# OpenPPL/ppl.llm.serving

Measured on AMD Instinct MI355X. Metric: decode tokens/sec, LLaMA-7B int8 (W8A16), max-running-batch 1024, higher is better.
Workload: dtype fp16 activations, int8 weights (W8A16), int8-g8 KV, fp32 accumulate

## Files before the change

include/pplhip.h:

```cpp
#ifndef PPLHIP_H_
#define PPLHIP_H_

#include <stdint.h>
#include <stddef.h>

#ifdef __cplusplus
extern "C" {
#endif

#define PPLHIP_API __attribute__((visibility("default")))

typedef enum pplhip_status {
    PPLHIP_SUCCESS = 0,
    PPLHIP_OTHER_ERROR = -1,
    PPLHIP_INVALID_VALUE = -2,
    PPLHIP_OUT_OF_MEMORY = -3,
    PPLHIP_DEVICE_RUNTIME_ERROR = -4,
    PPLHIP_DEVICE_MEMORY_ERROR = -5,
    PPLHIP_NOT_FOUND = -6,
    PPLHIP_UNSUPPORTED = -7
} pplhip_status;

typedef struct pplhip_model_desc {
    int32_t hidden_dim;
// ... 358 lines not shown


PPLHIP_API int pplhip_op_rmsnorm_form(int64_t rows, int32_t hidden, int32_t quant, int32_t wide_max_rows, char* buf, int32_t len);

PPLHIP_API int pplhip_op_rmsnorm_ex(void* stream, const void* x, const void* skip, const void* w, float eps, int64_t rows, int32_t hidden,
                                    const int64_t* gather_seq_starts, void* out, void* residual_out, void* q, float* sx, int32_t q_fp8,
                                    const float* slab_ws, int32_t slab_splits, const void* slab_scale, int64_t slab_M);

PPLHIP_API int pplhip_op_gather_last_rows(void* stream, const void* x, const int64_t* seq_starts, int64_t B, int32_t hidden, void* out);

PPLHIP_API int pplhip_op_rope_kv_write_ex(void* stream, void* qkv, const float* cos_sin, const pplhip_kv_view* kv, const int64_t* seq_starts,
                                          const int64_t* start_pos, const int64_t* cache_indices, int64_t max_pages, int64_t B, int64_t t0,
                                          int64_t T, int32_t num_heads, const float* slab_ws, int32_t slab_splits, const void* slab_scale,
                                          int64_t slab_M);

PPLHIP_API int pplhip_op_linear_defer(void* stream, const void* x, const void* w, const void* scale, int32_t wq_bit, int32_t group,
                                      int64_t M, int32_t N, int32_t K, void* y, int64_t ldy, void* ws, uint64_t ws_bytes, int32_t dry_run,
                                      int32_t* splits, const void** slab_scale, char* route, int32_t route_len);

PPLHIP_API int pplhip_op_attention(void* stream, const void* qkv, const pplhip_kv_view* kv,
                                   const int64_t* seq_starts, const int64_t* start_pos,
                                   const int64_t* cache_indices, int64_t max_pages, int64_t B, int64_t T,
                                   int64_t decoding_batches, int64_t max_seq_len, int64_t max_kv_len,
                                   int32_t num_heads, int32_t split_k, void* workspace, uint64_t workspace_bytes,
                                   void* out);

enum { PPLHIP_COMM_ALLREDUCE = 0, PPLHIP_COMM_ALLREDUCE_NORM = 1, PPLHIP_COMM_ALLGATHER = 2 };
typedef struct pplhip_comm_item {
    int32_t kind, channel;
    uint32_t epoch_advance;
// ... 28 lines not shown
```

ppl.llm.serving_amd/csrc/k_attn_decode.hip:

```cpp
#include <stdlib.h>
#include <hip/hip_ext.h>
#include "k_attn_decode_dev.h"

namespace pplhip {

template <int QBIT, int D>
__global__ void attn_decode_kernel(const uint16_t* __restrict__ qkv, KvAddr kv, const int64_t* __restrict__ seq_starts,
                                   const int64_t* __restrict__ start_pos, const int64_t* __restrict__ cache_indices,
                                   int64_t max_pages, int H, int Hkv, int split, float* __restrict__ workspace,
                                   uint16_t* __restrict__ out) {
    extern __shared__ __attribute__((aligned(16))) float smem[];
    attn_decode_body<QBIT, D>(qkv, kv, seq_starts, start_pos, cache_indices, max_pages, H, Hkv, split, workspace, out, (int)blockIdx.x,
                              (int64_t)blockIdx.y, (int)blockIdx.z, (int)(blockDim.x >> 6), smem);
}

template <int D>
__global__ void attn_decode_reduce_kernel(const float* __restrict__ workspace, int split, uint16_t* __restrict__ out) {
    const int64_t bh = blockIdx.x;
    const float* ws = workspace + bh * (int64_t)split * (D + 2);
    for (int d = threadIdx.x; d < D; d += blockDim.x) {
        const LseRow r = lse_merge(ws, split, D + 2, D, d);
        out[bh * D + d] = f2h(r.o / r.l);
    }
}

hipError_t launch_attn_reduce(hipStream_t s, const float* ws, int nsplit, int64_t n_row_heads, int D, uint16_t* out) {
    if (D != 128 && D != 64 && D != 32) return hipErrorInvalidValue;
    dispatch_int<128, 64, 32>(D, [&](auto DD) {
        hipLaunchKernelGGL((attn_decode_reduce_kernel<DD>), dim3((unsigned)n_row_heads), dim3(DD < 64 ? 64 : DD), 0, s, ws, nsplit, out);
    });
    return hipGetLastError();
}

size_t attn_decode_workspace_bytes(int64_t nb, int H, int D, int split) {
    return split > 1 ? (size_t)nb * H * split * (D + 2) * sizeof(float) : 0;
}

template <int QBIT, int D>
static hipError_t launch_decode_t(hipStream_t s, const uint16_t* qkv, const KvAddr& kv, const int64_t* seq_starts,
                                  const int64_t* start_pos, const int64_t* cache_indices, int64_t max_pages, int64_t nb,
                                  int H, int Hkv, int split, int threads, float* workspace, uint16_t* out, hipEvent_t t0,
                                  hipEvent_t t1) {
    const int nw = threads / 64;
    const size_t lds = (size_t)nw * (D + 2) * sizeof(float);
    if (t0 && t1)
        hipExtLaunchKernelGGL((attn_decode_kernel<QBIT, D>), dim3(H, (unsigned)nb, split), dim3(threads), lds, s, t0, t1, 0, qkv, kv,
                              seq_starts, start_pos, cache_indices, max_pages, H, Hkv, split, workspace, out);
    else
        hipLaunchKernelGGL((attn_decode_kernel<QBIT, D>), dim3(H, (unsigned)nb, split), dim3(threads), lds, s, qkv, kv,
                           seq_starts, start_pos, cache_indices, max_pages, H, Hkv, split, workspace, out);
    const hipError_t e = hipGetLastError();
    if (e != hipSuccess || split == 1) return e;
    return launch_attn_reduce(s, workspace, split, nb * H, D, out);
}

hipError_t launch_attn_decode(hipStream_t s, const uint16_t* qkv, const KvAddr& kv, int kv_fmt,
                              const int64_t* seq_starts, const int64_t* start_pos, const int64_t* cache_indices,
                              int64_t max_pages, int64_t nb, int H, int Hkv, int D, int64_t max_kv_len, int split,
                              int threads, float* workspace, uint16_t* out, hipEvent_t t0, hipEvent_t t1) {
    if (nb == 0) return hipSuccess;
    static const int forced_tpb = tune_int("PPLHIP_ATTN_TPB", 0);
    if (forced_tpb) threads = forced_tpb;
    if (threads < 64 || threads > 64 * DEC_MAX_WAVES || threads % 64) return hipErrorInvalidValue;
    if (threads < D) threads = D;
    if (split < 1) split = 1;
    static const bool no_gqa = tune_set("PPLHIP_ATTN_NOGQA");
    if (attn_decode_gqa_supported(kv_fmt, H, Hkv, D) && !no_gqa) {
        hipError_t e = launch_attn_decode_gqa(s, qkv, kv, kv_fmt, seq_starts, start_pos, cache_indices, max_pages, nb, H,
                                              Hkv, D, split, workspace, out, t0, t1);
        if (e != hipSuccess || split == 1) return e;
        return launch_attn_reduce(s, workspace, split, nb * H, D, out);
    }
    if ((kv_fmt != KV_FP16 && kv_fmt != KV_I8G8 && kv_fmt != KV_FP8 && kv_fmt != KV_I4G32) || (D != 128 && D != 64 && D != 32)) return hipErrorInvalidValue;
    hipError_t e = hipSuccess;
    dispatch_int<KV_I8G8, KV_FP16, KV_FP8, KV_I4G32>(kv_fmt, [&](auto QB) {
        dispatch_int<128, 64, 32>(D, [&](auto DD) {
            e = launch_decode_t<QB, DD>(s, qkv, kv, seq_starts, start_pos, cache_indices, max_pages, nb, H, Hkv, split, threads, workspace,
                                        out, t0, t1);
        });
    });
    return e;
}

}
```

ppl.llm.serving_amd/csrc/k_attn_decode_dev.h:

```cpp
#pragma once
#include "k_attn_dev.h"

namespace pplhip {

constexpr int DEC_UNROLL = 4;
constexpr int DEC_MAX_WAVES = 8;

template <int QBIT, int D>
__device__ __forceinline__ void attn_decode_body(const uint16_t* __restrict__ qkv, const KvAddr& kv, const int64_t* __restrict__ seq_starts,
                                                 const int64_t* __restrict__ start_pos, const int64_t* __restrict__ cache_indices,
                                                 int64_t max_pages, int H, int Hkv, int split, float* __restrict__ workspace,
                                                 uint16_t* __restrict__ out, int hq, int64_t b, int sp, int nw, float* smem) {
    using C = AttnCfg<QBIT, D>;
    constexpr int CH = C::CH, LPT = C::LPT, TPW = C::TPW;

    const int hk = hq / (H / Hkv);
    const int lane = threadIdx.x & 63;
    const int wave = threadIdx.x >> 6;
    const int g = lane / LPT;
    const int c = lane - g * LPT;
    const int ch0 = c * CH;

    const int64_t kv_len = start_pos[b] + 1;
    const int64_t per = (kv_len + split - 1) / split;
    const int64_t tbeg = sp * per;
    const int64_t tend = (tbeg + per < kv_len) ? tbeg + per : kv_len;

    const uint16_t* qrow = qkv + seq_starts[b] * (int64_t)(H + 2 * Hkv) * D + (int64_t)hq * D + ch0;
    float q[CH];
    if constexpr (CH == 32) {
#pragma unroll
        for (int i = 0; i < 4; ++i) unpack8(*reinterpret_cast<const uint4*>(qrow + 8 * i), q + 8 * i);
    } else if constexpr (CH == 16) {
        unpack8(*reinterpret_cast<const uint4*>(qrow), q);
        unpack8(*reinterpret_cast<const uint4*>(qrow + 8), q + 8);
    } else {
        unpack8(*reinterpret_cast<const uint4*>(qrow), q);
    }
    float qsum[C::NG > 0 ? C::NG : 1];
    if constexpr (QBIT == 8) {
#pragma unroll
        for (int gi = 0; gi < C::NG; ++gi) {
            float s = 0.f;
#pragma unroll
            for (int i = 0; i < 8; ++i) s += q[gi * 8 + i];
            qsum[gi] = s * 128.0f;
        }
    }
    if constexpr (QBIT == KV_I4G32) {
        float s = 0.f;
#pragma unroll
        for (int i = 0; i < CH; ++i) s += q[i];
// ... 223 lines not shown
```

ppl.llm.serving_amd/csrc/k_rope_kv.hip:

```cpp
#include <stdlib.h>
#include "kernels.h"

namespace pplhip {

template <int QBIT>
__device__ __forceinline__ void store_group8(const KvAddr& kv, int kvsel, int head, int64_t slot, int ch0,
                                             const float* x ) {
    const int64_t base = (int64_t)kvsel * kv.sKV + (int64_t)head * kv.sH + slot * kv.sN + ch0;
    if constexpr (QBIT == 0) {
        *reinterpret_cast<uint4*>(reinterpret_cast<uint16_t*>(kv.cache) + base) = pack8(x);
    } else {
        float mx = 0.f;
#pragma unroll
        for (int i = 0; i < 8; ++i) mx = fmaxf(mx, fabsf(x[i]));
        const _Float16 sh = to_h(mx / 127.0f);
        const float sf = (float)sh;
        const float inv = sf > 0.f ? __fdiv_rn(1.0f, sf) : 0.f;
        uint32_t lo = 0, hi = 0;
#pragma unroll
        for (int i = 0; i < 8; ++i) {
            float q = rintf(__fmul_rn(x[i], inv));
            q = fminf(fmaxf(q, -127.f), 127.f);
            const uint32_t b = (uint32_t)(int)q & 0xffu;
            if (i < 4) lo |= b << (8 * i); else hi |= b << (8 * (i - 4));
// ... 13 lines not shown
#pragma unroll
    for (int i = 0; i < 8; ++i) {
        const float y = __fmul_rn(x[i], inv);
        const uint32_t b = fp8_e4m3_rne(fminf(fmaxf(y, -lim), lim));
        if (i < 4) lo |= b << (8 * i); else hi |= b << (8 * (i - 4));
    }
    *reinterpret_cast<uint2*>(reinterpret_cast<uint8_t*>(kv.cache) + base) = make_uint2(lo, hi);
    if (ch0 == 0) kv.scale[(int64_t)kvsel * kv.ssKV + (int64_t)head * kv.ssH + slot * kv.ssN] = f2h(__builtin_bit_cast(float, (uint32_t)(127 + e) << 23));
}
__device__ __forceinline__ void store_i4_group8(const KvAddr& kv, int kvsel, int head, int64_t slot, int ch0, const float* x , float amax) {
    const float sf = kv_i4_scale(amax);
    const float inv = __fdiv_rn(1.0f, sf);
    const int64_t base = (int64_t)kvsel * kv.sKV + (int64_t)head * kv.sH + slot * kv.sN + ch0 / 2;
    *reinterpret_cast<uint32_t*>(reinterpret_cast<uint8_t*>(kv.cache) + base) = kv_i4_pack8(x, inv);
    if ((ch0 & 31) == 0) kv.scale[(int64_t)kvsel * kv.ssKV + (int64_t)head * kv.ssH + slot * kv.ssN + ch0 / 32] = f2h(sf);
}
__device__ __forceinline__ float group_max(float v, int n) {
    for (int o = 1; o < n; o <<= 1) v = fmaxf(v, __shfl_xor(v, o, 64));
    return v;
}

template <int QBIT>
__global__ __launch_bounds__(256) void rope_kv_write_kernel(uint16_t* __restrict__ qkv, const float* __restrict__ cos_sin,
                                                            KvAddr kv, const int64_t* __restrict__ seq_starts,
                                                            const int64_t* __restrict__ start_pos,
                                                            const int64_t* __restrict__ cache_indices, int64_t max_pages,
                                                            int64_t B, int64_t t0, int H, int Hkv, int D, SplitSlabs sl) {
    const int64_t t = t0 + blockIdx.x;
    int64_t b;
    {
// ... 22 lines not shown
        if (w < n_rope) {
            const int head = w / bph, i0 = (w - head * bph) * 8;
            uint16_t* x = row + (int64_t)head * D;
            float a[8], bb[8], c[8], s[8], ra[8], rb[8];
            if (sl.splits) {
                slab_load8(sl, t - t0, head * D + i0, a);
                slab_load8(sl, t - t0, head * D + i0 + half, bb);
            } else {
                unpack8(*reinterpret_cast<const uint4*>(x + i0), a);
                unpack8(*reinterpret_cast<const uint4*>(x + i0 + half), bb);
            }
            *reinterpret_cast<float4*>(c) = *reinterpret_cast<const float4*>(cs + i0);
            *reinterpret_cast<float4*>(c + 4) = *reinterpret_cast<const float4*>(cs + i0 + 4);
            *reinterpret_cast<float4*>(s) = *reinterpret_cast<const float4*>(cs + half + i0);
            *reinterpret_cast<float4*>(s + 4) = *reinterpret_cast<const float4*>(cs + half + i0 + 4);
#pragma unroll
            for (int i = 0; i < 8; ++i) {
                ra[i] = round_h(__fsub_rn(__fmul_rn(a[i], c[i]), __fmul_rn(bb[i], s[i])));
                rb[i] = round_h(__fadd_rn(__fmul_rn(bb[i], c[i]), __fmul_rn(a[i], s[i])));
            }
            if (head < H) {
                *reinterpret_cast<uint4*>(x + i0) = pack8(ra);
                *reinterpret_cast<uint4*>(x + i0 + half) = pack8(rb);
            } else if constexpr (QBIT == KV_FP8) {
                float mx = 0.f;
#pragma unroll
                for (int i = 0; i < 8; ++i) mx = fmaxf(mx, fmaxf(fabsf(ra[i]), fabsf(rb[i])));
                const int e = fp8_row_exp(group_max(mx, bph));
                store_fp8_row8(kv, 0, head - H, slot, i0, ra, e);
                store_fp8_row8(kv, 0, head - H, slot, i0 + half, rb, e);
            } else if constexpr (QBIT == KV_I4G32) {
                float ma = 0.f, mb = 0.f;
#pragma unroll
                for (int i = 0; i < 8; ++i) { ma = fmaxf(ma, fabsf(ra[i])); mb = fmaxf(mb, fabsf(rb[i])); }
                if (D == 32) ma = mb = group_max(fmaxf(ma, mb), 2);
// ... 15 lines not shown
#pragma unroll
                for (int i = 0; i < 8; ++i) mx = fmaxf(mx, fabsf(v[i]));
                store_fp8_row8(kv, 1, head, slot, i0, v, fp8_row_exp(group_max(mx, D / 8)));
            } else if constexpr (QBIT == KV_I4G32) {
                float mx = 0.f;
#pragma unroll
                for (int i = 0; i < 8; ++i) mx = fmaxf(mx, fabsf(v[i]));
                store_i4_group8(kv, 1, head, slot, i0, v, group_max(mx, 4));
            } else {
                store_group8<QBIT>(kv, 1, head, slot, i0, v);
            }
        }
    }
}

hipError_t launch_rope_kv_write(hipStream_t s, uint16_t* qkv, const float* cos_sin, const KvAddr& kv, int kv_fmt, const int64_t* seq_starts, const int64_t* start_pos,
                                const int64_t* cache_indices, int64_t max_pages, int64_t B, int64_t t0, int64_t T, int H,
                                int Hkv, int D, const SplitSlabs* qkv_slabs) {
    if (T == 0) return hipSuccess;
    SplitSlabs sl;
    if (qkv_slabs && qkv_slabs->splits > 0) {
        sl = *qkv_slabs;
        if (sl.N != (H + 2 * Hkv) * D || sl.M != T) return hipErrorInvalidValue;
    }
    if (D % 16 || (kv_fmt != KV_FP16 && kv_fmt != KV_I8G8 && kv_fmt != KV_FP8 && kv_fmt != KV_I4G32)) return hipErrorInvalidValue;
    if (kv_fmt == KV_I4G32 && D != 32 && D != 64 && D != 128) return hipErrorInvalidValue;
    const int items = (H + Hkv) * (D / 16) + Hkv * (D / 8);
    static const int forced_y = getenv("PPLHIP_ROPE_BLOCKS_PER_TOKEN") ? atoi(getenv("PPLHIP_ROPE_BLOCKS_PER_TOKEN")) : 0;
    int gy = (items + 255) / 256;
    if (gy > 4) gy = 4;
    if (T >= 4096 && gy > 2) gy = 2;
    if (forced_y > 0) gy = forced_y;
    const dim3 grid((unsigned)T, (unsigned)gy);
    if (kv_fmt == KV_I4G32)
        hipLaunchKernelGGL(rope_kv_write_kernel<KV_I4G32>, grid, dim3(256), 0, s, qkv, cos_sin, kv, seq_starts,
                           start_pos, cache_indices, max_pages, B, t0, H, Hkv, D, sl);
    else if (kv_fmt == KV_FP8)
        hipLaunchKernelGGL(rope_kv_write_kernel<KV_FP8>, grid, dim3(256), 0, s, qkv, cos_sin, kv, seq_starts,
                           start_pos, cache_indices, max_pages, B, t0, H, Hkv, D, sl);
    else if (kv_fmt == KV_I8G8)
        hipLaunchKernelGGL(rope_kv_write_kernel<8>, grid, dim3(256), 0, s, qkv, cos_sin, kv, seq_starts,
                           start_pos, cache_indices, max_pages, B, t0, H, Hkv, D, sl);
    else
// ... 7 lines not shown
```

ppl.llm.serving_amd/csrc/kernels.h:

```cpp
#pragma once
#include <hip/hip_runtime.h>
#include <stdint.h>
#include "k_common.h"

namespace pplhip {

struct SplitSlabs {
    const float* ws = nullptr;
    int splits = 0;
    const uint16_t* scale = nullptr;
    int N = 0;
    int64_t M = 0;
};
struct LinearRoute {
    char* buf = nullptr;
    int cap = 0;
    int len = 0;
    bool dry = false;
    void add(const char* fmt, ...) __attribute__((format(printf, 2, 3)));
};
inline const char* epi_name(int epi) { return epi == 1 ? "f32" : (epi == 2 ? "swiglu" : "f16"); }
#ifdef __HIPCC__
__device__ __forceinline__ void slab_load8(const SplitSlabs& sl, int64_t m, int n, float* o) {
    const float* p = sl.ws + m * sl.N + n;
// ... 29 lines not shown
                          int64_t rows, int hidden, const int64_t* gather_seq_starts, uint16_t* out,
                          uint16_t* residual_out, int8_t* qout = nullptr, float* sx = nullptr,
                          const SplitSlabs* skip_slabs = nullptr,
                          bool q_fp8 = false);
struct RmsnormForm {
    int maxc = 0, nt = 0;
};
hipError_t rmsnorm_form(int64_t rows, int hidden, int wide_max_rows, RmsnormForm* f);
int rmsnorm_wide_max_rows();
hipError_t launch_silu_mul(hipStream_t s, const uint16_t* gate_up, int64_t T, int inter, uint16_t* out);
hipError_t launch_gather_last_rows(hipStream_t s, const uint16_t* x, const int64_t* seq_starts, int64_t B, int hidden, uint16_t* out);

hipError_t launch_rope_kv_write(hipStream_t s, uint16_t* qkv, const float* cos_sin, const KvAddr& kv, int kv_fmt,
                                const int64_t* seq_starts, const int64_t* start_pos,
                                const int64_t* cache_indices, int64_t max_pages, int64_t B, int64_t t0, int64_t T, int H,
                                int Hkv, int D, const SplitSlabs* qkv_slabs = nullptr);

size_t attn_decode_workspace_bytes(int64_t nb, int H, int D, int split);
hipError_t launch_attn_decode(hipStream_t s, const uint16_t* qkv, const KvAddr& kv, int kv_fmt,
                              const int64_t* seq_starts, const int64_t* start_pos, const int64_t* cache_indices,
                              int64_t max_pages, int64_t nb, int H, int Hkv, int D, int64_t max_kv_len, int split,
                              int threads, float* workspace, uint16_t* out, hipEvent_t t0 = nullptr, hipEvent_t t1 = nullptr);
hipError_t launch_attn_reduce(hipStream_t s, const float* ws, int nsplit, int64_t n_row_heads, int D, uint16_t* out);

hipError_t launch_attn_prefill(hipStream_t s, const uint16_t* qkv, const KvAddr& kv, int kv_fmt,
                               const int64_t* seq_starts, const int64_t* start_pos, const int64_t* cache_indices,
                               int64_t max_pages, int64_t b0, int64_t B, int H, int Hkv, int D, int64_t max_seq_len,
                               uint16_t* out, int64_t max_kv_len = 0, float* ws = nullptr, size_t ws_bytes = 0, int64_t row0 = 0,
                               int64_t nrows = 0);

hipError_t launch_attn_prefill32(hipStream_t s, const uint16_t* qkv, const KvAddr& kv, int kv_fmt, const int64_t* seq_starts,
                                 const int64_t* start_pos, const int64_t* cache_indices, int64_t max_pages, int64_t b0, int64_t B,
                                 int H, int Hkv, int D, int64_t max_seq_len, uint16_t* out, int64_t max_kv_len = 0, float* ws = nullptr,
                                 size_t ws_bytes = 0, int64_t row0 = 0, int64_t nrows = 0);

bool attn_decode_gqa_supported(int kv_fmt, int H, int Hkv, int D);
hipError_t launch_attn_decode_gqa(hipStream_t s, const uint16_t* qkv, const KvAddr& kv, int kv_fmt,
// ... 127 lines not shown
```

ppl.llm.serving_amd/csrc/pplhip.cc:

```cpp
#include "rt_internal.h"

bool verbose() {
    static const bool on = getenv("PPLHIP_VERBOSE") != nullptr;
    return on;
}

void comm_note(pplhip_ctx* c, const std::string& msg) {
    fprintf(stderr, "[pplhip] %s\n", msg.c_str());
    if (c) { if (!c->comm_notes.empty()) c->comm_notes += "; "; c->comm_notes += msg; }
}

int fail(pplhip_ctx* c, int rank, int code, const std::string& msg) {
    if (c) {
        if (rank >= 0 && rank < (int)c->ranks.size()) c->ranks[rank].err = msg; else c->err = msg;
    }
    if (verbose()) fprintf(stderr, "[pplhip] error %d (rank %d): %s\n", code, rank, msg.c_str());
    return code;
}

static inline float h2f_host(uint16_t h) { return (float)__builtin_bit_cast(_Float16, h); }
static inline uint16_t f2h_host(float f) { return __builtin_bit_cast(uint16_t, (_Float16)f); }

static int act_format(int act_quant_bit, int weight_quant_bit) {
    if (act_quant_bit == 0) return ACT_FP16;
// ... 903 lines not shown
               !sh.capturing) {
        const int64_t bm = B >= 64 ? (B / 2 + 15) / 16 * 16 : B / 2;
        p.chunk[0] = Chunk{0, bm, 0, bm, bm};
        p.chunk[1] = Chunk{bm, B - bm, bm, B - bm, B - bm};
        p.schedule = SCHED_TWO_LANES;
        p.lane1_ws_off = bm * (int64_t)s.heads * 32 * (s.head_dim + 2);
    }
    p.num_chunks = p.schedule == SCHED_ONE_LANE ? 1 : 2;
    for (int i = 0; i < 2; ++i) p.decode_split[i] = i < p.num_chunks && p.chunk[i].nd > 0 ? decode_split(s, p.chunk[i].nd, sh.max_kv_len) : 1;
    p.fuse_norm = fuse_norm_active(s, dump);
    p.defer_qkv = s.defer_on && s.act_fmt == ACT_FP16 && !dump && p.schedule != SCHED_TWO_CHUNKS && !sh.lora;
    p.defer_reduce = p.defer_qkv && !comm;
    return p;
}

Lane make_lane(Rank& R, int i, int64_t attn_ws_off) {
    Lane ln;
    ln.stream = i ? R.stream2 : R.stream;
    ln.gemm_ws = i ? R.gemm_ws2 : R.gemm_ws;
    ln.attn_ws = R.attn_ws + attn_ws_off;
    ln.attn_ws_bytes = R.attn_ws_bytes - (size_t)attn_ws_off * 4;
    ln.ch = &R.ch[i];
    return ln;
}

static int layer_linear(pplhip_ctx* c, int rank, Lane& lane, const Linear& l, const uint16_t* x, int64_t M, void* y, int64_t ldy, bool swiglu,
                        bool pre_quantised = false, SplitSlabs* defer = nullptr) {
    Rank& R = c->ranks[rank];
    hipStream_t s = lane.stream;
    if (c->act_fmt == ACT_FP8) {
// ... 31 lines not shown
    Layer& L = R.layers[l];
    ProfEvent ev;
    uint16_t* h = R.h + k.t0 * hd;
    uint16_t* xn = R.xn + k.t0 * hd;
    const bool a8 = c->act_fmt != ACT_FP16;
    if (!xn_ready)
        HIPCK(c, rank, launch_rmsnorm(s, h, pending ? pending + k.t0 * hd : nullptr, L.attn_norm, d.norm_eps, k.tn, hd, nullptr, xn,
                                      pending ? h : nullptr, a8 ? R.xq : nullptr, a8 ? R.sx : nullptr, pending ? &lane.sl_part2 : nullptr,
                                      c->act_fmt == ACT_FP8));
    lane.sl_part2 = SplitSlabs{};
    prof_begin(c, R, lane, PPLHIP_PROF_GEMM, &ev);
    if (int rc = layer_linear(c, rank, lane, L.wqkv, xn, k.tn, R.qkv + k.t0 * nqkv, L.wqkv.N, false, a8, p.defer_qkv ? &lane.sl_qkv : nullptr)) return rc;
    prof_end(R, lane, &ev);
    if (int rc = layer_lora(c, rank, lane, l, LORA_WQKV, R.xn, hd, R.qkv, nqkv, hd)) return rc;
    const KvAddr kv = make_kv_addr(d, Hkv, D, R.kv_tokens, R.kv_cache, R.kv_scale, l);
    HIPCK(c, rank, launch_rope_kv_write(s, R.qkv, R.rope, kv, c->kv_fmt, R.d_seq, R.d_sp, R.d_ci,
                                        R.max_pages, R.B, k.t0, k.tn, H, Hkv, D, &lane.sl_qkv));
    lane.sl_qkv = SplitSlabs{};
    const int64_t ci_stride = d.cache_mode == 1 ? R.max_pages : 1;
    if (k.nd > 0) {
        const bool light = c->o.enable_profiling == 2;
        prof_begin(c, R, lane, PPLHIP_PROF_ATTN_DECODE, &ev);
        if (light) {
            std::pair<hipEvent_t, hipEvent_t> pr;
            if (!R.prof_free.empty()) { pr = R.prof_free.back(); R.prof_free.pop_back(); }
            else { hipEventCreate(&pr.first); hipEventCreate(&pr.second); }
            ev.cls = PPLHIP_PROF_ATTN_DECODE; ev.a = pr.first; ev.b = pr.second;
        }
        HIPCK(c, rank, launch_attn_decode(s, R.qkv, kv, c->kv_fmt, R.d_seq + k.b0, R.d_sp + k.b0, R.d_ci + k.b0 * ci_stride,
                                          R.max_pages, k.nd, H, Hkv, D, R.max_kv_len, split, threads, lane.attn_ws,
                                          R.att + k.b0 * (int64_t)H * D, light ? ev.a : nullptr, light ? ev.b : nullptr));
        if (light) R.prof.push_back(ev);
        else prof_end(R, lane, &ev);
    }
    if (k.bn > k.nd) {
        prof_begin(c, R, lane, PPLHIP_PROF_ATTN_PREFILL, &ev);
        HIPCK(c, rank, launch_attn_prefill(s, R.qkv, kv, c->kv_fmt, R.d_seq, R.d_sp, R.d_ci, R.max_pages, k.b0 + k.nd,
                                           k.b0 + k.bn, H, Hkv, D, R.max_seq_len, R.att, R.max_kv_len, lane.attn_ws, lane.attn_ws_bytes,
                                           k.t0 + k.nd, k.tn - k.nd));
        prof_end(R, lane, &ev);
    }
    prof_begin(c, R, lane, PPLHIP_PROF_GEMM, &ev);
    if (int rc = layer_linear(c, rank, lane, L.wo, R.att + k.t0 * (int64_t)H * D, k.tn, R.part + k.t0 * hd, hd, false, false,
                              p.defer_reduce ? &lane.sl_part : nullptr))
        return rc;
    prof_end(R, lane, &ev);
// ... 320 lines not shown
```

ppl.llm.serving_amd/csrc/rt_internal.h:

```cpp
#pragma once
#include "../../include/pplhip.h"

#include <hip/hip_runtime.h>
#include <rccl/rccl.h>

#include <algorithm>
#include <cmath>
#include <cstdio>
#include <cstdlib>
#include <cstring>
#include <map>
#include <unordered_map>
#include <memory>
#include <string>
#include <vector>

#include "kernels.h"

using namespace pplhip;

enum { ACT_FP16 = 0, ACT_I8 = 1, ACT_FP8 = 2 };

struct Linear {
    int N = 0, K = 0, qbit = 0, group = 0;
// ... 313 lines not shown
            return fail(c, r, PPLHIP_DEVICE_RUNTIME_ERROR, std::string(#expr) + ": " + ncclGetErrorString(e__));     \
    } while (0)

bool verbose();
void comm_note(pplhip_ctx* c, const std::string& msg);
int fail(pplhip_ctx* c, int rank, int code, const std::string& msg);
int dev_alloc(pplhip_ctx* c, int r, void** p, uint64_t bytes);
int kv_format(int quant_bit, int quant_group, int D);
KvAddr make_kv_addr(const pplhip_model_desc& d, int Hkv, int D, uint64_t tokens, void* cache, uint16_t* scale, int layer);
using Chunk = pplhip_chunk;
using StepPlan = pplhip_step_plan;
pplhip_plan_settings plan_settings(const pplhip_ctx* c, const Rank& R);
bool fuse_norm_active(const pplhip_plan_settings& s, bool dump);
StepPlan plan_step(const pplhip_plan_settings& s, const pplhip_step_shape& sh);
Lane make_lane(Rank& R, int i, int64_t attn_ws_off);
int chunk_allreduce(pplhip_ctx* c, int rank, Lane& lane, uint16_t* buf, const Chunk& k, int ci, bool overlapped, const uint16_t* norm_w = nullptr);
int p2p_connect_local(pplhip_ctx* c);
int p2p_check(pplhip_ctx* c, int rank);
int p2p_next_epoch(pplhip_ctx* c, int rank, Channel& ch, hipStream_t s, uint32_t* epoch);
void lora_build_tiles(const int32_t* row_slots, int64_t T, std::vector<LoraTile>& out);
int sample_row_list(const int32_t* top_k, int B, int32_t* rows);
int top_logprobs_row_list(const int32_t* num_logprobs, int B, int32_t* rows);
int run_prompt_logprobs(pplhip_ctx* c, int rank, hipStream_t s, const uint16_t* pending, const SplitSlabs& sl_part2);
```

ppl.llm.serving_amd/csrc/rt_ops.cc:

```cpp
#include "rt_internal.h"

static int op_rc(hipError_t e) { return e == hipSuccess ? 0 : (e == hipErrorInvalidValue ? PPLHIP_INVALID_VALUE : PPLHIP_DEVICE_RUNTIME_ERROR); }

int pplhip_op_embedding(void* stream, const int64_t* token_ids, const void* table, int64_t T, int32_t hidden, void* out) {
    return op_rc(launch_embedding((hipStream_t)stream, token_ids, (const uint16_t*)table, T, hidden, (uint16_t*)out));
}

int pplhip_op_rmsnorm(void* stream, const void* x, const void* skip, const void* w, float eps, int64_t T, int32_t hidden,
                      void* out, void* residual_out) {
    return op_rc(launch_rmsnorm((hipStream_t)stream, (const uint16_t*)x, (const uint16_t*)skip, (const uint16_t*)w, eps, T,
                                hidden, nullptr, (uint16_t*)out, (uint16_t*)residual_out));
}

static float* op_linear_ws(size_t* bytes) {
    static float* ws[16] = {nullptr};
    static const size_t ws_bytes = (size_t)64 << 20;
    int dev = 0;
    *bytes = 0;
    if (hipGetDevice(&dev) != hipSuccess || dev < 0 || dev >= 16) return nullptr;
    if (!ws[dev] && hipMalloc((void**)&ws[dev], ws_bytes) != hipSuccess) ws[dev] = nullptr;
    if (ws[dev]) *bytes = ws_bytes;
    return ws[dev];
}

// ... 323 lines not shown
    if (B < 0 || (B > 0 && (!x || !seq_starts || !out))) return PPLHIP_INVALID_VALUE;
    return op_rc(launch_gather_last_rows((hipStream_t)stream, (const uint16_t*)x, seq_starts, B, hidden, (uint16_t*)out));
}

int pplhip_op_rope_kv_write_ex(void* stream, void* qkv, const float* cos_sin, const pplhip_kv_view* kv, const int64_t* seq_starts,
                               const int64_t* start_pos, const int64_t* cache_indices, int64_t max_pages, int64_t B, int64_t t0, int64_t T,
                               int32_t num_heads, const float* slab_ws, int32_t slab_splits, const void* slab_scale, int64_t slab_M) {
    const int fmt = kv ? kv_format(kv->quant_bit, kv->quant_group, kv->head_dim) : -1;
    if (fmt < 0 || t0 < 0 || T < 0 || B < 0) return PPLHIP_INVALID_VALUE;
    SplitSlabs sl;
    if (!op_slabs(slab_ws, slab_splits, slab_scale, slab_M, (num_heads + 2 * kv->kv_heads) * kv->head_dim, &sl)) return PPLHIP_INVALID_VALUE;
    return op_rc(launch_rope_kv_write((hipStream_t)stream, (uint16_t*)qkv, cos_sin, view_addr(kv), fmt, seq_starts, start_pos, cache_indices,
                                      max_pages, B, t0, T, num_heads, kv->kv_heads, kv->head_dim, &sl));
}

int pplhip_op_linear_defer(void* stream, const void* x, const void* w, const void* scale, int32_t wq_bit, int32_t group, int64_t M, int32_t N,
                           int32_t K, void* y, int64_t ldy, void* ws, uint64_t ws_bytes, int32_t dry_run, int32_t* splits,
                           const void** slab_scale, char* route, int32_t route_len) {
    LinearRoute r;
    r.buf = route_len > 0 ? route : nullptr;
    r.cap = route_len;
    r.dry = dry_run != 0;
    if (r.buf) r.buf[0] = 0;
    SplitSlabs sl;
    const hipError_t e = launch_linear((hipStream_t)stream, (const uint16_t*)x, w, (const uint16_t*)scale, wq_bit, group, M, N, K, y, ldy, false,
                                       (float*)ws, (size_t)ws_bytes, false, &sl, &r);
    if (splits) *splits = sl.splits;
    if (slab_scale) *slab_scale = sl.scale;
    return op_rc(e);
}
// ... 25 lines not shown
```

ppl.llm.serving_amd/pplhip.py:

```python
import ctypes as C
import os
import struct
import subprocess

import numpy as np

_DIR = os.path.dirname(os.path.abspath(__file__))
LIB_PATH = os.environ.get("PPLHIP_LIB") or os.path.join(_DIR, "csrc", "libpplhip.so")
UNIQUE_ID_BYTES = 128
IPC_HANDLE_BYTES = 64
COMM_NONE, COMM_RCCL, COMM_P2P = 0, 1, 2
_LIB = None

STATUS = {0: "SUCCESS", -1: "OTHER_ERROR", -2: "INVALID_VALUE", -3: "OUT_OF_MEMORY", -4: "DEVICE_RUNTIME_ERROR",
          -5: "DEVICE_MEMORY_ERROR", -6: "NOT_FOUND", -7: "UNSUPPORTED"}

PROF_ATTN_DECODE, PROF_ATTN_PREFILL, PROF_GEMM, PROF_RUN, PROF_LORA = 0, 1, 2, 3, 4


class PplHipError(RuntimeError):
    pass


class ModelDesc(C.Structure):
# ... 137 lines not shown

SYMBOLS = [
    "pplhip_version", "pplhip_device_count", "pplhip_get_unique_id", "pplhip_init", "pplhip_destroy",
    "pplhip_comm_export", "pplhip_comm_connect", "pplhip_comm_mode", "pplhip_comm_fused_norm", "pplhip_comm_info", "pplhip_comm_allreduce_us", "pplhip_comm_op",
    "pplhip_last_error", "pplhip_rank_load", "pplhip_rank_set_tensor", "pplhip_rank_init_synthetic", "pplhip_rank_tie_output",
    "pplhip_kv_block_bytes", "pplhip_kv_capacity", "pplhip_kv_alloc", "pplhip_kv_ptrs", "pplhip_kv_read",
    "pplhip_kv_write", "pplhip_kv_fill_synthetic",
    "pplhip_lora_set_tensor", "pplhip_lora_commit", "pplhip_lora_load", "pplhip_lora_unload", "pplhip_set_adapters", "pplhip_op_lora",
    "pplhip_set_inputs", "pplhip_set_prompt_logprobs", "pplhip_prompt_logprobs", "pplhip_run", "pplhip_debug_run_dump", "pplhip_logits", "pplhip_copy_logits", "pplhip_sync",
    "pplhip_sample", "pplhip_sample_rows", "pplhip_top_logprobs", "pplhip_logit_rule_set", "pplhip_logit_edit", "pplhip_guide_set_vocab", "pplhip_guide_load", "pplhip_guide_unload", "pplhip_guide_edit", "pplhip_penalty", "pplhip_profile_reset", "pplhip_profile_get", "pplhip_profile_mode", "pplhip_mem_info",
    "pplhip_op_embedding", "pplhip_op_rmsnorm", "pplhip_op_linear", "pplhip_op_linear_swiglu", "pplhip_op_linear_ex", "pplhip_op_step_plan", "pplhip_op_rmsnorm_quant", "pplhip_op_quant_act", "pplhip_op_quant_weight",
    "pplhip_op_linear_i8", "pplhip_op_rmsnorm_quant_f8", "pplhip_op_quant_act_f8", "pplhip_op_quant_weight_f8", "pplhip_op_linear_f8",
    "pplhip_op_silu_mul", "pplhip_op_penalty", "pplhip_op_sample", "pplhip_op_sample_rows", "pplhip_op_sample_uniform", "pplhip_op_top_logprobs", "pplhip_op_prompt_logprobs", "pplhip_op_logit_edit", "pplhip_op_guide_build", "pplhip_op_guide_mask", "pplhip_op_rope_kv_write",
    "pplhip_op_attention", "pplhip_build_rope_table",
    "pplhip_op_rmsnorm_form", "pplhip_op_rmsnorm_ex", "pplhip_op_gather_last_rows", "pplhip_op_rope_kv_write_ex", "pplhip_op_linear_defer",
]


def build():
    subprocess.check_call(["make", "-s", "-j8", "-C", os.path.join(_DIR, "csrc")])


def lib():
    global _LIB
    if _LIB is None:
        if not os.path.exists(LIB_PATH):
            raise PplHipError(f"{LIB_PATH} is missing: build it with __graft_entry__.build() (no CPU fallback exists)")
        L = C.CDLL(LIB_PATH)
        vp, i32, i64, u64, f32 = C.c_void_p, C.c_int32, C.c_int64, C.c_uint64, C.c_float
        L.pplhip_last_error.restype = C.c_char_p
# ... 79 lines not shown
            L.pplhip_guide_unload.argtypes = [vp, i32]
            L.pplhip_guide_edit.argtypes = [vp, vp, C.POINTER(GuideEditArgs)]
            L.pplhip_op_guide_build.argtypes = [vp, vp, vp, i32, vp, vp, i32, vp, i32, i32, vp, i64, vp]
            L.pplhip_op_guide_mask.argtypes = [vp, vp, i32, i32, i32, vp, vp, vp, i32, i32, i64, vp, i32]
        L.pplhip_op_rope_kv_write.argtypes = [vp, vp, vp, C.POINTER(KvView), vp, vp, vp, i64, i64, i64, i32]
        L.pplhip_op_attention.argtypes = [vp, vp, C.POINTER(KvView), vp, vp, vp, i64, i64, i64, i64, i64, i64, i32, i32,
                                          vp, u64, vp]
        L.pplhip_build_rope_table.argtypes = [vp, i32, i32, f32]
        if hasattr(L, "pplhip_op_rmsnorm_form"):
            L.pplhip_op_rmsnorm_form.argtypes = [i64, i32, i32, i32, C.c_char_p, i32]
            L.pplhip_op_rmsnorm_ex.argtypes = [vp, vp, vp, vp, f32, i64, i32, vp, vp, vp, vp, vp, i32, vp, i32, vp, i64]
            L.pplhip_op_gather_last_rows.argtypes = [vp, vp, vp, i64, i32, vp]
            L.pplhip_op_rope_kv_write_ex.argtypes = [vp, vp, vp, C.POINTER(KvView), vp, vp, vp, i64, i64, i64, i64, i32, vp, i32, vp, i64]
            L.pplhip_op_linear_defer.argtypes = [vp, vp, vp, vp, i32, i32, i64, i32, i32, vp, i64, vp, u64, i32, C.POINTER(i32), C.POINTER(vp),
                                                 C.c_char_p, i32]
        _LIB = L
    return _LIB


def linear_route(x, w, scale, wq_bit, group, M, N, K, y, ldy, epi, ws=None, ws_bytes=0, dry_run=True, stream=None):
    buf = C.create_string_buffer(1024)
    rc = lib().pplhip_op_linear_ex(stream, x, w, scale, wq_bit, group, M, N, K, y, ldy, epi, ws, ws_bytes, int(dry_run), buf, 1024)
    return rc, buf.value.decode()


def rmsnorm_form(rows, hidden, quant=0, wide_max_rows=512):
    buf = C.create_string_buffer(64)
    rc = lib().pplhip_op_rmsnorm_form(rows, hidden, quant, wide_max_rows, buf, 64)
    return rc, buf.value.decode()

# ... 528 lines not shown
```

Measured before the change: 23980.

## Fuse Q RoPE rotation into decode attention and add decode-specialized rope/KV-write kernel

Adds a decode-only rope/KV-write kernel that can skip rotating Q heads. It assigns per-token parts with unrolled loads and resolves the KV slot once per wave. The decode attention kernel now applies the rotary rotation to Q itself when loading the query row, so Q is not written back and re-read. The fused path is on by default, gated by an env toggle, and limited to the non-GQA fp16 and int8-g8 paths. It adds cos/sin and partner-half loads inside the attention kernel. LLaMA-7B is MHA, so the fused-Q path applies here.

```diff
diff --git a/include/pplhip.h b/include/pplhip.h
--- a/include/pplhip.h
+++ b/include/pplhip.h
@@ -396,6 +396,16 @@
                                           int64_t T, int32_t num_heads, const float* slab_ws, int32_t slab_splits, const void* slab_scale,
                                           int64_t slab_M);
 
+PPLHIP_API int pplhip_op_rope_kv_write_decode(void* stream, void* qkv, const float* cos_sin, const pplhip_kv_view* kv,
+                                              const int64_t* seq_starts, const int64_t* start_pos, const int64_t* cache_indices,
+                                              int64_t max_pages, int64_t B, int64_t t0, int64_t T, int32_t num_heads, int64_t b0,
+                                              int32_t skip_q);
+PPLHIP_API int pplhip_op_attention_decode_rot(void* stream, const void* qkv, const float* cos_sin, const pplhip_kv_view* kv,
+                                              const int64_t* seq_starts, const int64_t* start_pos, const int64_t* cache_indices,
+                                              int64_t max_pages, int64_t nb, int64_t max_kv_len, int32_t num_heads, int32_t split_k,
+                                              void* workspace, uint64_t workspace_bytes, void* out);
+PPLHIP_API int pplhip_op_attn_rotate_q(int32_t set);
+
 PPLHIP_API int pplhip_op_linear_defer(void* stream, const void* x, const void* w, const void* scale, int32_t wq_bit, int32_t group,
                                       int64_t M, int32_t N, int32_t K, void* y, int64_t ldy, void* ws, uint64_t ws_bytes, int32_t dry_run,
                                       int32_t* splits, const void** slab_scale, char* route, int32_t route_len);
diff --git a/ppl.llm.serving_amd/csrc/k_attn_decode.hip b/ppl.llm.serving_amd/csrc/k_attn_decode.hip
--- a/ppl.llm.serving_amd/csrc/k_attn_decode.hip
+++ b/ppl.llm.serving_amd/csrc/k_attn_decode.hip
@@ -8,10 +8,10 @@
 __global__ void attn_decode_kernel(const uint16_t* __restrict__ qkv, KvAddr kv, const int64_t* __restrict__ seq_starts,
                                    const int64_t* __restrict__ start_pos, const int64_t* __restrict__ cache_indices,
                                    int64_t max_pages, int H, int Hkv, int split, float* __restrict__ workspace,
-                                   uint16_t* __restrict__ out) {
+                                   uint16_t* __restrict__ out, const float* __restrict__ rope_q) {
     extern __shared__ __attribute__((aligned(16))) float smem[];
     attn_decode_body<QBIT, D>(qkv, kv, seq_starts, start_pos, cache_indices, max_pages, H, Hkv, split, workspace, out, (int)blockIdx.x,
-                              (int64_t)blockIdx.y, (int)blockIdx.z, (int)(blockDim.x >> 6), smem);
+                              (int64_t)blockIdx.y, (int)blockIdx.z, (int)(blockDim.x >> 6), smem, rope_q);
 }
 
 template <int D>
@@ -40,25 +40,32 @@
 static hipError_t launch_decode_t(hipStream_t s, const uint16_t* qkv, const KvAddr& kv, const int64_t* seq_starts,
                                   const int64_t* start_pos, const int64_t* cache_indices, int64_t max_pages, int64_t nb,
                                   int H, int Hkv, int split, int threads, float* workspace, uint16_t* out, hipEvent_t t0,
-                                  hipEvent_t t1) {
+                                  hipEvent_t t1, const float* rope_q) {
     const int nw = threads / 64;
     const size_t lds = (size_t)nw * (D + 2) * sizeof(float);
     if (t0 && t1)
         hipExtLaunchKernelGGL((attn_decode_kernel<QBIT, D>), dim3(H, (unsigned)nb, split), dim3(threads), lds, s, t0, t1, 0, qkv, kv,
-                              seq_starts, start_pos, cache_indices, max_pages, H, Hkv, split, workspace, out);
+                              seq_starts, start_pos, cache_indices, max_pages, H, Hkv, split, workspace, out, rope_q);
     else
         hipLaunchKernelGGL((attn_decode_kernel<QBIT, D>), dim3(H, (unsigned)nb, split), dim3(threads), lds, s, qkv, kv,
-                           seq_starts, start_pos, cache_indices, max_pages, H, Hkv, split, workspace, out);
+                           seq_starts, start_pos, cache_indices, max_pages, H, Hkv, split, workspace, out, rope_q);
     const hipError_t e = hipGetLastError();
     if (e != hipSuccess || split == 1) return e;
     return launch_attn_reduce(s, workspace, split, nb * H, D, out);
 }
 
+bool attn_decode_rotates_q(int kv_fmt, int H, int Hkv, int D) {
+    static const bool no_gqa = tune_set("PPLHIP_ATTN_NOGQA");
+    if (attn_decode_gqa_supported(kv_fmt, H, Hkv, D) && !no_gqa) return false;
+    return (kv_fmt == KV_FP16 || kv_fmt == KV_I8G8) && (D == 128 || D == 64 || D == 32);
+}
+
 hipError_t launch_attn_decode(hipStream_t s, const uint16_t* qkv, const KvAddr& kv, int kv_fmt,
                               const int64_t* seq_starts, const int64_t* start_pos, const int64_t* cache_indices,
                               int64_t max_pages, int64_t nb, int H, int Hkv, int D, int64_t max_kv_len, int split,
-                              int threads, float* workspace, uint16_t* out, hipEvent_t t0, hipEvent_t t1) {
+                              int threads, float* workspace, uint16_t* out, hipEvent_t t0, hipEvent_t t1, const float* rope_q) {
     if (nb == 0) return hipSuccess;
+    if (rope_q && !attn_decode_rotates_q(kv_fmt, H, Hkv, D)) return hipErrorInvalidValue;
     static const int forced_tpb = tune_int("PPLHIP_ATTN_TPB", 0);
     if (forced_tpb) threads = forced_tpb;
     if (threads < 64 || threads > 64 * DEC_MAX_WAVES || threads % 64) return hipErrorInvalidValue;
@@ -76,7 +83,7 @@
     dispatch_int<KV_I8G8, KV_FP16, KV_FP8, KV_I4G32>(kv_fmt, [&](auto QB) {
         dispatch_int<128, 64, 32>(D, [&](auto DD) {
             e = launch_decode_t<QB, DD>(s, qkv, kv, seq_starts, start_pos, cache_indices, max_pages, nb, H, Hkv, split, threads, workspace,
-                                        out, t0, t1);
+                                        out, t0, t1, rope_q);
         });
     });
     return e;
diff --git a/ppl.llm.serving_amd/csrc/k_attn_decode_dev.h b/ppl.llm.serving_amd/csrc/k_attn_decode_dev.h
--- a/ppl.llm.serving_amd/csrc/k_attn_decode_dev.h
+++ b/ppl.llm.serving_amd/csrc/k_attn_decode_dev.h
@@ -10,7 +10,8 @@
 __device__ __forceinline__ void attn_decode_body(const uint16_t* __restrict__ qkv, const KvAddr& kv, const int64_t* __restrict__ seq_starts,
                                                  const int64_t* __restrict__ start_pos, const int64_t* __restrict__ cache_indices,
                                                  int64_t max_pages, int H, int Hkv, int split, float* __restrict__ workspace,
-                                                 uint16_t* __restrict__ out, int hq, int64_t b, int sp, int nw, float* smem) {
+                                                 uint16_t* __restrict__ out, int hq, int64_t b, int sp, int nw, float* smem,
+                                                 const float* __restrict__ rope_q = nullptr) {
     using C = AttnCfg<QBIT, D>;
     constexpr int CH = C::CH, LPT = C::LPT, TPW = C::TPW;
 
@@ -36,6 +37,27 @@
         unpack8(*reinterpret_cast<const uint4*>(qrow + 8), q + 8);
     } else {
         unpack8(*reinterpret_cast<const uint4*>(qrow), q);
+    }
+    if constexpr (CH <= D / 2) {
+        if (rope_q) {
+            constexpr int half = D / 2;
+            const bool lo = ch0 < half;
+            const uint16_t* prow = lo ? qrow + half : qrow - half;
+            const float* cs = rope_q + start_pos[b] * D + (lo ? ch0 : ch0 - half);
+            float pr[CH], cc[CH], sn[CH];
+#pragma unroll
+            for (int i = 0; i < CH / 8; ++i) unpack8(*reinterpret_cast<const uint4*>(prow + 8 * i), pr + 8 * i);
+#pragma unroll
+            for (int i = 0; i < CH / 4; ++i) {
+                *reinterpret_cast<float4*>(cc + 4 * i) = *reinterpret_cast<const float4*>(cs + 4 * i);
+                *reinterpret_cast<float4*>(sn + 4 * i) = *reinterpret_cast<const float4*>(cs + half + 4 * i);
+            }
+#pragma unroll
+            for (int i = 0; i < CH; ++i) {
+                const float own = __fmul_rn(q[i], cc[i]), par = __fmul_rn(pr[i], sn[i]);
+                q[i] = round_h(lo ? __fsub_rn(own, par) : __fadd_rn(own, par));
+            }
+        }
     }
     float qsum[C::NG > 0 ? C::NG : 1];
     if constexpr (QBIT == 8) {
diff --git a/ppl.llm.serving_amd/csrc/k_rope_kv.hip b/ppl.llm.serving_amd/csrc/k_rope_kv.hip
--- a/ppl.llm.serving_amd/csrc/k_rope_kv.hip
+++ b/ppl.llm.serving_amd/csrc/k_rope_kv.hip
@@ -51,6 +51,13 @@
     const int64_t base = (int64_t)kvsel * kv.sKV + (int64_t)head * kv.sH + slot * kv.sN + ch0 / 2;
     *reinterpret_cast<uint32_t*>(reinterpret_cast<uint8_t*>(kv.cache) + base) = kv_i4_pack8(x, inv);
     if ((ch0 & 31) == 0) kv.scale[(int64_t)kvsel * kv.ssKV + (int64_t)head * kv.ssH + slot * kv.ssN + ch0 / 32] = f2h(sf);
+}
+__device__ __forceinline__ void rotate8(const float* a, const float* b, const float* c, const float* s, float* ra, float* rb) {
+#pragma unroll
+    for (int i = 0; i < 8; ++i) {
+        ra[i] = round_h(__fsub_rn(__fmul_rn(a[i], c[i]), __fmul_rn(b[i], s[i])));
+        rb[i] = round_h(__fadd_rn(__fmul_rn(b[i], c[i]), __fmul_rn(a[i], s[i])));
+    }
 }
 __device__ __forceinline__ float group_max(float v, int n) {
     for (int o = 1; o < n; o <<= 1) v = fmaxf(v, __shfl_xor(v, o, 64));
@@ -103,11 +110,7 @@
             *reinterpret_cast<float4*>(c + 4) = *reinterpret_cast<const float4*>(cs + i0 + 4);
             *reinterpret_cast<float4*>(s) = *reinterpret_cast<const float4*>(cs + half + i0);
             *reinterpret_cast<float4*>(s + 4) = *reinterpret_cast<const float4*>(cs + half + i0 + 4);
-#pragma unroll
-            for (int i = 0; i < 8; ++i) {
-                ra[i] = round_h(__fsub_rn(__fmul_rn(a[i], c[i]), __fmul_rn(bb[i], s[i])));
-                rb[i] = round_h(__fadd_rn(__fmul_rn(bb[i], c[i]), __fmul_rn(a[i], s[i])));
-            }
+            rotate8(a, bb, c, s, ra, rb);
             if (head < H) {
                 *reinterpret_cast<uint4*>(x + i0) = pack8(ra);
                 *reinterpret_cast<uint4*>(x + i0 + half) = pack8(rb);
@@ -153,9 +156,94 @@
     }
 }
 
+constexpr int DU = 4;
+template <int QBIT>
+__global__ __launch_bounds__(256) void rope_kv_write_decode_kernel(uint16_t* __restrict__ qkv, const float* __restrict__ cos_sin, KvAddr kv,
+                                                                   const int64_t* __restrict__ start_pos,
+                                                                   const int64_t* __restrict__ cache_indices, int64_t max_pages, int64_t b0,
+                                                                   int64_t t0, int64_t T, int parts, int H, int Hkv, int D, int w_first) {
+    const int lane = threadIdx.x & 63;
+    const int64_t g = (int64_t)blockIdx.x * 4 + __builtin_amdgcn_readfirstlane((int)(threadIdx.x >> 6));
+    const int64_t i = g / parts;
+    const int part = (int)(g - i * parts);
+    if (i >= T) return;
+    const int half = D / 2;
+    const int bph = half / 8;
+    const int n_rope = (H + Hkv) * bph, n = n_rope + Hkv * (D / 8);
+    const int stride = 64 * parts;
+    uint16_t* row = qkv + (t0 + i) * (int64_t)(H + 2 * Hkv) * D;
+    const bool cs_once = 64 % bph == 0;
+    float c[8], s[8];
+    bool resolved = false, have_cs = false;
+    int64_t pos = 0, slot = 0;
+    for (int w0 = w_first + part * 64 + lane; w0 < n; w0 += stride * DU) {
+        uint4 xa[DU], xb[DU];
+#pragma unroll
+        for (int u = 0; u < DU; ++u) {
+            const int w = w0 + u * stride;
+            xa[u] = xb[u] = make_uint4(0, 0, 0, 0);
+            if (w < n_rope) {
+                const int head = w / bph, i0 = (w - head * bph) * 8;
+                xa[u] = *reinterpret_cast<const uint4*>(row + (int64_t)head * D + i0);
+                xb[u] = *reinterpret_cast<const uint4*>(row + (int64_t)head * D + i0 + half);
+            } else if (w < n) {
+                const int wv = w - n_rope;
+                const int head = wv / (D / 8), i0 = (wv - head * (D / 8)) * 8;
+                xa[u] = *reinterpret_cast<const uint4*>(row + (int64_t)(H + Hkv + head) * D + i0);
+            }
+        }
+        if (!resolved) {
+            pos = start_pos[b0 + i];
+            slot = kv_slot(kv, cache_indices, max_pages, b0 + i, pos);
+            resolved = true;
+        }
+#pragma unroll
+        for (int u = 0; u < DU; ++u) {
+            const int w = w0 + u * stride;
+            if (w < n_rope) {
+                const int head = w / bph, i0 = (w - head * bph) * 8;
+                if (!have_cs || !cs_once) {
+                    const float* cs = cos_sin + pos * D;
+                    *reinterpret_cast<float4*>(c) = *reinterpret_cast<const float4*>(cs + i0);
+                    *reinterpret_cast<float4*>(c + 4) = *reinterpret_cast<const float4*>(cs + i0 + 4);
+                    *reinterpret_cast<float4*>(s) = *reinterpret_cast<const float4*>(cs + half + i0);
+                    *reinterpret_cast<float4*>(s + 4) = *reinterpret_cast<const float4*>(cs + half + i0 + 4);
+                    have_cs = true;
+                }
+                float a[8], bb[8], ra[8], rb[8];
+                unpack8(xa[u], a);
+                unpack8(xb[u], bb);
+                rotate8(a, bb, c, s, ra, rb);
+                if (head < H) {
+                    *reinterpret_cast<uint4*>(row + (int64_t)head * D + i0) = pack8(ra);
+                    *reinterpret_cast<uint4*>(row + (int64_t)head * D + i0 + half) = pack8(rb);
+                } else {
+                    store_group8<QBIT>(kv, 0, head - H, slot, i0, ra);
+                    store_group8<QBIT>(kv, 0, head - H, slot, i0 + half, rb);
+                }
+            } else if (w < n) {
+                const int wv = w - n_rope;
+                const int head = wv / (D / 8), i0 = (wv - head * (D / 8)) * 8;
+                float v[8];
+                unpack8(xa[u], v);
+                store_group8<QBIT>(kv, 1, head, slot, i0, v);
+            }
+        }
+    }
+}
+
+static int rope_forced_blocks() {
+    static const int forced_y = getenv("PPLHIP_ROPE_BLOCKS_PER_TOKEN") ? atoi(getenv("PPLHIP_ROPE_BLOCKS_PER_TOKEN")) : 0;
+    return forced_y;
+}
+
+bool rope_decode_form(int kv_fmt, bool slabs, int64_t decode_b0) {
+    return decode_b0 >= 0 && rope_forced_blocks() <= 0 && !slabs && (kv_fmt == KV_I8G8 || kv_fmt == KV_FP16);
+}
+
 hipError_t launch_rope_kv_write(hipStream_t s, uint16_t* qkv, const float* cos_sin, const KvAddr& kv, int kv_fmt, const int64_t* seq_starts, const int64_t* start_pos,
                                 const int64_t* cache_indices, int64_t max_pages, int64_t B, int64_t t0, int64_t T, int H,
-                                int Hkv, int D, const SplitSlabs* qkv_slabs) {
+                                int Hkv, int D, const SplitSlabs* qkv_slabs, int64_t decode_b0, bool skip_q) {
     if (T == 0) return hipSuccess;
     SplitSlabs sl;
     if (qkv_slabs && qkv_slabs->splits > 0) {
@@ -165,7 +253,21 @@
     if (D % 16 || (kv_fmt != KV_FP16 && kv_fmt != KV_I8G8 && kv_fmt != KV_FP8 && kv_fmt != KV_I4G32)) return hipErrorInvalidValue;
     if (kv_fmt == KV_I4G32 && D != 32 && D != 64 && D != 128) return hipErrorInvalidValue;
     const int items = (H + Hkv) * (D / 16) + Hkv * (D / 8);
-    static const int forced_y = getenv("PPLHIP_ROPE_BLOCKS_PER_TOKEN") ? atoi(getenv("PPLHIP_ROPE_BLOCKS_PER_TOKEN")) : 0;
+    const int forced_y = rope_forced_blocks();
+    if (decode_b0 >= 0 && decode_b0 + T > B) return hipErrorInvalidValue;
+    if (skip_q && !rope_decode_form(kv_fmt, sl.splits > 0, decode_b0)) return hipErrorInvalidValue;
+    if (rope_decode_form(kv_fmt, sl.splits > 0, decode_b0)) {
+        const int w_first = skip_q ? H * (D / 16) : 0;
+        const int parts = (items - w_first + 64 * DU - 1) / (64 * DU);
+        const dim3 grid((unsigned)((T * parts + 3) / 4));
+        if (kv_fmt == KV_I8G8)
+            hipLaunchKernelGGL(rope_kv_write_decode_kernel<8>, grid, dim3(256), 0, s, qkv, cos_sin, kv, start_pos, cache_indices, max_pages,
+                               decode_b0, t0, T, parts, H, Hkv, D, w_first);
+        else
+            hipLaunchKernelGGL(rope_kv_write_decode_kernel<0>, grid, dim3(256), 0, s, qkv, cos_sin, kv, start_pos, cache_indices, max_pages,
+                               decode_b0, t0, T, parts, H, Hkv, D, w_first);
+        return hipGetLastError();
+    }
     int gy = (items + 255) / 256;
     if (gy > 4) gy = 4;
     if (T >= 4096 && gy > 2) gy = 2;
diff --git a/ppl.llm.serving_amd/csrc/kernels.h b/ppl.llm.serving_amd/csrc/kernels.h
--- a/ppl.llm.serving_amd/csrc/kernels.h
+++ b/ppl.llm.serving_amd/csrc/kernels.h
@@ -67,13 +67,18 @@
 hipError_t launch_rope_kv_write(hipStream_t s, uint16_t* qkv, const float* cos_sin, const KvAddr& kv, int kv_fmt,
                                 const int64_t* seq_starts, const int64_t* start_pos,
                                 const int64_t* cache_indices, int64_t max_pages, int64_t B, int64_t t0, int64_t T, int H,
-                                int Hkv, int D, const SplitSlabs* qkv_slabs = nullptr);
+                                int Hkv, int D, const SplitSlabs* qkv_slabs = nullptr,
+                                int64_t decode_b0 = -1,
+                                bool skip_q = false);
+bool rope_decode_form(int kv_fmt, bool slabs, int64_t decode_b0);
 
 size_t attn_decode_workspace_bytes(int64_t nb, int H, int D, int split);
 hipError_t launch_attn_decode(hipStream_t s, const uint16_t* qkv, const KvAddr& kv, int kv_fmt,
                               const int64_t* seq_starts, const int64_t* start_pos, const int64_t* cache_indices,
                               int64_t max_pages, int64_t nb, int H, int Hkv, int D, int64_t max_kv_len, int split,
-                              int threads, float* workspace, uint16_t* out, hipEvent_t t0 = nullptr, hipEvent_t t1 = nullptr);
+                              int threads, float* workspace, uint16_t* out, hipEvent_t t0 = nullptr, hipEvent_t t1 = nullptr,
+                              const float* rope_q = nullptr);
+bool attn_decode_rotates_q(int kv_fmt, int H, int Hkv, int D);
 hipError_t launch_attn_reduce(hipStream_t s, const float* ws, int nsplit, int64_t n_row_heads, int D, uint16_t* out);
 
 hipError_t launch_attn_prefill(hipStream_t s, const uint16_t* qkv, const KvAddr& kv, int kv_fmt,
diff --git a/ppl.llm.serving_amd/csrc/pplhip.cc b/ppl.llm.serving_amd/csrc/pplhip.cc
--- a/ppl.llm.serving_amd/csrc/pplhip.cc
+++ b/ppl.llm.serving_amd/csrc/pplhip.cc
@@ -1,4 +1,5 @@
 #include "rt_internal.h"
+#include <atomic>
 
 bool verbose() {
     static const bool on = getenv("PPLHIP_VERBOSE") != nullptr;
@@ -941,6 +942,11 @@
     return p;
 }
 
+int attn_rotate_q(int set) {
+    static std::atomic<int> on{getenv("PPLHIP_ATTN_ROTATE_Q") ? atoi(getenv("PPLHIP_ATTN_ROTATE_Q")) != 0 : 1};
+    return set == 0 || set == 1 ? on.exchange(set) : on.load();
+}
+
 Lane make_lane(Rank& R, int i, int64_t attn_ws_off) {
     Lane ln;
     ln.stream = i ? R.stream2 : R.stream;
@@ -1002,8 +1008,10 @@
     prof_end(R, lane, &ev);
     if (int rc = layer_lora(c, rank, lane, l, LORA_WQKV, R.xn, hd, R.qkv, nqkv, hd)) return rc;
     const KvAddr kv = make_kv_addr(d, Hkv, D, R.kv_tokens, R.kv_cache, R.kv_scale, l);
+    const int64_t dec_b0 = k.nd == k.tn && k.bn == k.tn ? k.b0 : -1;
+    const bool rot_q = attn_rotate_q(-1) && rope_decode_form(c->kv_fmt, lane.sl_qkv.splits > 0, dec_b0) && attn_decode_rotates_q(c->kv_fmt, H, Hkv, D);
     HIPCK(c, rank, launch_rope_kv_write(s, R.qkv, R.rope, kv, c->kv_fmt, R.d_seq, R.d_sp, R.d_ci,
-                                        R.max_pages, R.B, k.t0, k.tn, H, Hkv, D, &lane.sl_qkv));
+                                        R.max_pages, R.B, k.t0, k.tn, H, Hkv, D, &lane.sl_qkv, dec_b0, rot_q));
     lane.sl_qkv = SplitSlabs{};
     const int64_t ci_stride = d.cache_mode == 1 ? R.max_pages : 1;
     if (k.nd > 0) {
@@ -1017,7 +1025,8 @@
         }
         HIPCK(c, rank, launch_attn_decode(s, R.qkv, kv, c->kv_fmt, R.d_seq + k.b0, R.d_sp + k.b0, R.d_ci + k.b0 * ci_stride,
                                           R.max_pages, k.nd, H, Hkv, D, R.max_kv_len, split, threads, lane.attn_ws,
-                                          R.att + k.b0 * (int64_t)H * D, light ? ev.a : nullptr, light ? ev.b : nullptr));
+                                          R.att + k.b0 * (int64_t)H * D, light ? ev.a : nullptr, light ? ev.b : nullptr,
+                                          rot_q ? R.rope : nullptr));
         if (light) R.prof.push_back(ev);
         else prof_end(R, lane, &ev);
     }
diff --git a/ppl.llm.serving_amd/csrc/rt_internal.h b/ppl.llm.serving_amd/csrc/rt_internal.h
--- a/ppl.llm.serving_amd/csrc/rt_internal.h
+++ b/ppl.llm.serving_amd/csrc/rt_internal.h
@@ -351,6 +351,7 @@
 bool fuse_norm_active(const pplhip_plan_settings& s, bool dump);
 StepPlan plan_step(const pplhip_plan_settings& s, const pplhip_step_shape& sh);
 Lane make_lane(Rank& R, int i, int64_t attn_ws_off);
+int attn_rotate_q(int set);
 int chunk_allreduce(pplhip_ctx* c, int rank, Lane& lane, uint16_t* buf, const Chunk& k, int ci, bool overlapped, const uint16_t* norm_w = nullptr);
 int p2p_connect_local(pplhip_ctx* c);
 int p2p_check(pplhip_ctx* c, int rank);
diff --git a/ppl.llm.serving_amd/csrc/rt_ops.cc b/ppl.llm.serving_amd/csrc/rt_ops.cc
--- a/ppl.llm.serving_amd/csrc/rt_ops.cc
+++ b/ppl.llm.serving_amd/csrc/rt_ops.cc
@@ -361,6 +361,29 @@
                                       max_pages, B, t0, T, num_heads, kv->kv_heads, kv->head_dim, &sl));
 }
 
+int pplhip_op_rope_kv_write_decode(void* stream, void* qkv, const float* cos_sin, const pplhip_kv_view* kv, const int64_t* seq_starts,
+                                   const int64_t* start_pos, const int64_t* cache_indices, int64_t max_pages, int64_t B, int64_t t0, int64_t T,
+                                   int32_t num_heads, int64_t b0, int32_t skip_q) {
+    const int fmt = kv ? kv_format(kv->quant_bit, kv->quant_group, kv->head_dim) : -1;
+    if (fmt < 0 || t0 < 0 || T < 0 || B < 0 || b0 < 0) return PPLHIP_INVALID_VALUE;
+    return op_rc(launch_rope_kv_write((hipStream_t)stream, (uint16_t*)qkv, cos_sin, view_addr(kv), fmt, seq_starts, start_pos, cache_indices,
+                                      max_pages, B, t0, T, num_heads, kv->kv_heads, kv->head_dim, nullptr, b0, skip_q != 0));
+}
+
+int pplhip_op_attn_rotate_q(int32_t set) { return attn_rotate_q(set); }
+
+int pplhip_op_attention_decode_rot(void* stream, const void* qkv, const float* cos_sin, const pplhip_kv_view* kv, const int64_t* seq_starts,
+                                   const int64_t* start_pos, const int64_t* cache_indices, int64_t max_pages, int64_t nb, int64_t max_kv_len,
+                                   int32_t num_heads, int32_t split_k, void* workspace, uint64_t workspace_bytes, void* out) {
+    const int fmt = kv ? kv_format(kv->quant_bit, kv->quant_group, kv->head_dim) : -1;
+    if (fmt < 0 || nb < 0 || !cos_sin) return PPLHIP_INVALID_VALUE;
+    const int split = split_k < 1 ? 1 : split_k;
+    if (split > 1 && attn_decode_workspace_bytes(nb, num_heads, kv->head_dim, split) > workspace_bytes) return PPLHIP_INVALID_VALUE;
+    return op_rc(launch_attn_decode((hipStream_t)stream, (const uint16_t*)qkv, view_addr(kv), fmt, seq_starts, start_pos, cache_indices, max_pages,
+                                    nb, num_heads, kv->kv_heads, kv->head_dim, max_kv_len, split, 256, (float*)workspace, (uint16_t*)out, nullptr,
+                                    nullptr, cos_sin));
+}
+
 int pplhip_op_linear_defer(void* stream, const void* x, const void* w, const void* scale, int32_t wq_bit, int32_t group, int64_t M, int32_t N,
                            int32_t K, void* y, int64_t ldy, void* ws, uint64_t ws_bytes, int32_t dry_run, int32_t* splits,
                            const void** slab_scale, char* route, int32_t route_len) {
diff --git a/ppl.llm.serving_amd/pplhip.py b/ppl.llm.serving_amd/pplhip.py
--- a/ppl.llm.serving_amd/pplhip.py
+++ b/ppl.llm.serving_amd/pplhip.py
@@ -175,6 +175,7 @@
     "pplhip_op_silu_mul", "pplhip_op_penalty", "pplhip_op_sample", "pplhip_op_sample_rows", "pplhip_op_sample_uniform", "pplhip_op_top_logprobs", "pplhip_op_prompt_logprobs", "pplhip_op_logit_edit", "pplhip_op_guide_build", "pplhip_op_guide_mask", "pplhip_op_rope_kv_write",
     "pplhip_op_attention", "pplhip_build_rope_table",
     "pplhip_op_rmsnorm_form", "pplhip_op_rmsnorm_ex", "pplhip_op_gather_last_rows", "pplhip_op_rope_kv_write_ex", "pplhip_op_linear_defer",
+    "pplhip_op_rope_kv_write_decode", "pplhip_op_attention_decode_rot", "pplhip_op_attn_rotate_q",
 ]
 
 
@@ -284,6 +285,10 @@
             L.pplhip_op_rope_kv_write_ex.argtypes = [vp, vp, vp, C.POINTER(KvView), vp, vp, vp, i64, i64, i64, i64, i32, vp, i32, vp, i64]
             L.pplhip_op_linear_defer.argtypes = [vp, vp, vp, vp, i32, i32, i64, i32, i32, vp, i64, vp, u64, i32, C.POINTER(i32), C.POINTER(vp),
                                                  C.c_char_p, i32]
+        if hasattr(L, "pplhip_op_rope_kv_write_decode"):
+            L.pplhip_op_rope_kv_write_decode.argtypes = [vp, vp, vp, C.POINTER(KvView), vp, vp, vp, i64, i64, i64, i64, i32, i64, i32]
+            L.pplhip_op_attention_decode_rot.argtypes = [vp, vp, vp, C.POINTER(KvView), vp, vp, vp, i64, i64, i64, i32, i32, vp, u64, vp]
+            L.pplhip_op_attn_rotate_q.argtypes = [i32]
         _LIB = L
     return _LIB
 
```

New measurement: 23920. No clear change (-0.2%).
